# Aedelon/MASt3R-SLAM

Hardware: AMD Instinct MI355X
Metric: keyframe-pairs/sec (512x512 two-view infer+match+GN) (higher is better)
Workload: dtype fp16

## Files before the change

### mast3r-slam_amd/csrc/conv_tail.hip

```cpp
#include "gemm_common.h"

using namespace m3gemm;

namespace {

constexpr int kThreads = 512;
constexpr int TH = 16, TW = 32;
constexpr int HH = TH + 2, HW = TW + 2;
constexpr int kHaloPix = HH * HW;
constexpr int kHaloBytes = kHaloPix * 128;
constexpr int kWStage = 128 * 128;
constexpr int PH = 11, PW = 19;
constexpr int kPatchBytes = (PH * PW * 128 + 1023) / 1024 * 1024;
constexpr int kLdsBytes = kHaloBytes + 2 * kWStage + kPatchBytes;

struct TailArgs {
    const bf16_t *X;
    const bf16_t *Wc;
    const float *bias;
    const bf16_t *W4;
    const float *b4;
    float *pts, *conf;
    bf16_t *Y;
    const bf16_t *R;
    int cout, relu_in;
    const bf16_t *zero16;
    int B, H, W, IH, IW;
    const bf16_t *Wc2, *W42;
    const float *bias2, *b42;
};

enum { EP_PLAIN = 0 , EP_TAIL = 1 , EP_RELU = 2 ,
       EP_ADD = 3  };

template <int DT, bool UPS, int CIN, int EP>
__global__ void __launch_bounds__(kThreads, 2)
k_conv_tail(const TailArgs ain) {
    constexpr bool TAIL = EP == EP_TAIL;
    static_assert(CIN % 64 == 0 && (TAIL ? CIN == 128 : true), "64-channel steps; the fused tail is the 128-channel head.2");
    constexpr int NQ = CIN / 64;
    TailArgs a = ain;
    if (blockIdx.y == 1) {
        a.Wc = ain.Wc2; a.W4 = ain.W42; a.bias = ain.bias2; a.b4 = ain.b42;
        a.X = ain.X + (size_t)ain.B * ain.IH * ain.IW * CIN;
        if (TAIL) {
            a.pts = ain.pts + (size_t)ain.B * ain.H * ain.W * 3;
            a.conf = ain.conf + (size_t)ain.B * ain.H * ain.W;
        } else {
            a.Y = ain.Y + (size_t)ain.B * ain.H * ain.W * ain.cout;
            if (EP == EP_ADD) a.R = ain.R + (size_t)ain.B * ain.H * ain.W * ain.cout;
        }
    }
    if (!TAIL) {
        const int z = blockIdx.z;
        a.Wc += (size_t)z * 128 * 9 * CIN;
        if (a.bias) a.bias += z * 128;
        a.Y += z * 128;
        if (EP == EP_ADD) a.R += z * 128;
    }
    extern __shared__ __attribute__((aligned(16))) unsigned char lds[];
    unsigned char *halo = lds, *wst = lds + kHaloBytes, *patch = lds + kHaloBytes + 2 * kWStage;
    const int tid = threadIdx.x, lane = tid & 63, wave = tid >> 6;
    const int wp = wave >> 1, wc = wave & 1;
    const int tiles_x = (a.W + TW - 1) / TW, tiles_y = a.H / TH;
    const int nwg = tiles_x * tiles_y * a.B;
    const int bid = xcd_remap(blockIdx.x, nwg);
    const int b = bid / (tiles_x * tiles_y), trem = bid - b * tiles_x * tiles_y;
    const int ty = trem / tiles_x, tx = trem - ty * tiles_x;
    const int oy0 = ty * TH, ox0 = tx * TW;
    const bf16_t *img = a.X + (size_t)b * a.IH * a.IW * CIN;

    auto stage_w = [&](int tap, int half, int buf) {
        unsigned char *base = wst + buf * kWStage;
#pragma unroll
        for (int i = 0; i < 2; ++i) {
            const int slot = i * kThreads + tid;
            const int row = slot >> 3, cp = slot & 7;
            const int c = half * 8 + (cp ^ ((row >> 1) & 7));
            glds16(a.Wc + ((size_t)row * 9 + tap) * CIN + c * 8, base + i * (kThreads * 16) + wave * 1024);
        }
    };
    const float sy = UPS && a.H > 1 ? (float)(a.IH - 1) / (float)(a.H - 1) : 0.f;
    const float sx = UPS && a.W > 1 ? (float)(a.IW - 1) / (float)(a.W - 1) : 0.f;
    const int py0 = (int)((float)max(oy0 - 1, 0) * sy), px0 = (int)((float)max(ox0 - 1, 0) * sx);
    auto stage_patch = [&](int half) {
        for (int wi = wave; wi < (PH * PW * 8 + 63) / 64; wi += kThreads / 64) {
            int slot = wi * 64 + lane;
            slot = slot < PH * PW * 8 ? slot : PH * PW * 8 - 1;
            const int pp = slot >> 3, c = slot & 7;
            const int y = min(py0 + pp / PW, a.IH - 1), x = min(px0 + pp % PW, a.IW - 1);
            glds16(img + ((size_t)y * a.IW + x) * CIN + (half * 8 + c) * 8, patch + wi * 1024);
        }
    };
    auto stage_halo_direct = [&](int half) {
        for (int wi = wave; wi < (kHaloPix * 8 + 63) / 64; wi += kThreads / 64) {
            int slot = wi * 64 + lane;
            const bool live = slot < kHaloPix * 8;
            slot = live ? slot : kHaloPix * 8 - 1;
            const int pix = slot >> 3, cp = slot & 7;
            const int hy = pix / HW, hx = pix - hy * HW;
            const int iy = oy0 + hy - 1, ix = ox0 + hx - 1;
            const int c = half * 8 + (cp ^ ((hx >> 1) & 7));
            const bool in = iy >= 0 && iy < a.H && ix >= 0 && ix < a.W;
            const void *src = in ? (const void *)(img + ((size_t)iy * a.IW + ix) * CIN + c * 8) : (const void *)a.zero16;
            if (wi * 64 + 64 <= kHaloPix * 8) glds16(src, halo + wi * 1024);
            else if (live) *reinterpret_cast<uint4 *>(halo + (size_t)slot * 16) = *reinterpret_cast<const uint4 *>(src);
        }
    };
    auto blend_halo = [&]() {
        for (int slot = tid; slot < kHaloPix * 8; slot += kThreads) {
            const int pix = slot >> 3, cp = slot & 7;
            const int hy = pix / HW, hx = pix - hy * HW;
            const int iy = oy0 + hy - 1, ix = ox0 + hx - 1;
            const int c = cp ^ ((hx >> 1) & 7);
            uint4 o = make_uint4(0u, 0u, 0u, 0u);
            if (iy >= 0 && iy < a.H && ix >= 0 && ix < a.W) {
                const float fy = iy * sy, fx = ix * sx;
                int y0 = (int)fy, x0 = (int)fx;
                y0 = min(y0, a.IH - 1); x0 = min(x0, a.IW - 1);
                const int y1 = min(y0 + 1, a.IH - 1), x1 = min(x0 + 1, a.IW - 1);
                const float wy = fy - (float)y0, wx = fx - (float)x0;
                const unsigned char *p = patch + c * 16;
                union U { uint4 q; unsigned w[4]; } q00, q01, q10, q11, r;
                q00.q = *reinterpret_cast<const uint4 *>(p + ((y0 - py0) * PW + (x0 - px0)) * 128);
                q01.q = *reinterpret_cast<const uint4 *>(p + ((y0 - py0) * PW + (x1 - px0)) * 128);
                q10.q = *reinterpret_cast<const uint4 *>(p + ((y1 - py0) * PW + (x0 - px0)) * 128);
                q11.q = *reinterpret_cast<const uint4 *>(p + ((y1 - py0) * PW + (x1 - px0)) * 128);
#pragma unroll
                for (int k = 0; k < 4; ++k) {
                    const float tl = lo16<DT>(q00.w[k]) * (1.f - wx) + lo16<DT>(q01.w[k]) * wx;
                    const float bl = lo16<DT>(q10.w[k]) * (1.f - wx) + lo16<DT>(q11.w[k]) * wx;
                    const float th = hi16<DT>(q00.w[k]) * (1.f - wx) + hi16<DT>(q01.w[k]) * wx;
                    const float bh = hi16<DT>(q10.w[k]) * (1.f - wx) + hi16<DT>(q11.w[k]) * wx;
                    r.w[k] = pack16<DT>(tl * (1.f - wy) + bl * wy, th * (1.f - wy) + bh * wy);
                }
                o = r.q;
            }
            *reinterpret_cast<uint4 *>(halo + (size_t)slot * 16) = o;
        }
    };

    f32x4 acc[8][4];
#pragma unroll
    for (int i = 0; i < 8; ++i)
#pragma unroll
        for (int j = 0; j < 4; ++j) acc[i][j] = f32x4{0.f, 0.f, 0.f, 0.f};
    const int frow = lane & 15, fch = lane >> 4;
    int w_off[4];
#pragma unroll
    for (int j = 0; j < 4; ++j) {
        const int r = wc * 64 + j * 16 + frow;
        w_off[j] = r * 128 + ((fch ^ ((r >> 1) & 7)) << 4);
    }

    const int group = wave >> 2;
    bf16x8 af[8], wf[4];
    const int pix_of_row = (int)((0x3D9F2A40E6C851B7ULL >> (4 * frow)) & 15);
    auto col_offset = [&](int hx) { return hx * 128 + ((fch ^ ((hx >> 1) & 7)) << 4); };
    auto read_frags = [&](int g, int tap, int ks) {
        const int ky = tap / 3, kx = tap - ky * 3;
        const unsigned char *wsrc = wst + (g & 1) * kWStage;
        const int flip = ks << 6;
        const int c0 = col_offset(pix_of_row + kx) ^ flip;
        const int c1 = col_offset(16 + pix_of_row + kx) ^ flip;
        const unsigned char *rowp = halo + (wp * 4 + ky) * (HW * 128);
#pragma unroll
        for (int j = 0; j < 4; ++j) wf[j] = *reinterpret_cast<const bf16x8 *>(wsrc + (w_off[j] ^ flip));
#pragma unroll
        for (int i = 0; i < 8; ++i)
            af[i] = *reinterpret_cast<const bf16x8 *>(rowp + (i >> 1) * (HW * 128) + ((i & 1) ? c1 : c0));
        if (!TAIL && a.relu_in) {
#pragma unroll
            for (int i = 0; i < 8; ++i) af[i] = relu_frag(af[i]);
        }
    };
    auto mfma_all = [&]() {
        __builtin_amdgcn_s_setprio(1);
#pragma unroll
        for (int i = 0; i < 8; ++i)
#pragma unroll
            for (int j = 0; j < 4; ++j) acc[i][j] = mfma16<DT>(wf[j], af[i], acc[i][j]);
        __builtin_amdgcn_s_setprio(0);
    };
    auto phase_end = [&]() {
        __builtin_amdgcn_sched_barrier(0);
        __builtin_amdgcn_s_barrier();
        __builtin_amdgcn_sched_barrier(0);
    };
    auto phase_end_wait = [&]() {
        __builtin_amdgcn_sched_barrier(0);
        asm volatile("s_waitcnt vmcnt(0)" ::: "memory");
        __builtin_amdgcn_s_barrier();
        __builtin_amdgcn_sched_barrier(0);
    };
    auto prefetch_w = [&](int g) { if (g + 1 < 9 * NQ) stage_w((g + 1) % 9, (g + 1) / 9, (g + 1) & 1); };
    auto run_half = [&](int half) {
        if (group == 0) {
#pragma unroll 1
            for (int tap = 0; tap < 9; ++tap) {
                const int g = half * 9 + tap;
                read_frags(g, tap, 0);
                prefetch_w(g);
                asm volatile("s_waitcnt lgkmcnt(0)" ::: "memory");
                phase_end();
                mfma_all();
                phase_end();
                read_frags(g, tap, 1);
                asm volatile("s_waitcnt lgkmcnt(0)" ::: "memory");
                phase_end();
                mfma_all();
                phase_end_wait();
            }
            phase_end();
        } else {
#pragma unroll 1
            for (int tap = 0; tap < 9; ++tap) {
                const int g = half * 9 + tap;
                if (tap > 0) mfma_all();
                phase_end();
                read_frags(g, tap, 0);
                prefetch_w(g);
                asm volatile("s_waitcnt lgkmcnt(0)" ::: "memory");
                phase_end();
                mfma_all();
                phase_end();
                read_frags(g, tap, 1);
                asm volatile("s_waitcnt lgkmcnt(0)" ::: "memory");
                phase_end_wait();
            }
            mfma_all();
            phase_end();
        }
    };

    stage_w(0, 0, 0);
    if (UPS) stage_patch(0); else stage_halo_direct(0);
    asm volatile("s_waitcnt vmcnt(0)" ::: "memory");
    lds_barrier();
#pragma unroll 1
    for (int q = 0; q < NQ; ++q) {
        if (UPS) {
            blend_halo();
            lds_barrier();
            if (q + 1 < NQ) stage_patch(q + 1);
        } else if (q > 0) {
            stage_halo_direct(q);
            asm volatile("s_waitcnt vmcnt(0)" ::: "memory");
            lds_barrier();
        }
        run_half(q);
    }

    if constexpr (EP == EP_ADD) {
        const int r = lane & 15, gq = lane >> 4;
        constexpr int RS = 272;
        unsigned char *wl = halo + wave * (32 * RS);
        float4 bj[4];
#pragma unroll
        for (int j = 0; j < 4; ++j)
            bj[j] = a.bias ? *reinterpret_cast<const float4 *>(a.bias + wc * 64 + j * 16 + gq * 4) : make_float4(0.f, 0.f, 0.f, 0.f);
        auto pix = [&](int pass, int rl, int &oy, int &ox) {
            const int i = pass * 2 + (rl >> 4);
            oy = oy0 + wp * 4 + (i >> 1);
            ox = ox0 + (i & 1) * 16 + (int)((0x3D9F2A40E6C851B7ULL >> (4 * (rl & 15))) & 15);
        };
        uint4 q[2][4];
        auto load_resid = [&](int pass, uint4 (&dst)[4]) {
#pragma unroll
            for (int it = 0; it < 4; ++it) {
                const int c = it * 64 + lane, rl = c >> 3, ch = c & 7;
                int oy, ox;
                pix(pass, rl, oy, ox);
                ox = ox < a.W ? ox : a.W - 1;
                dst[it] = *reinterpret_cast<const uint4 *>(a.R + (((size_t)b * a.H + oy) * a.W + ox) * a.cout + wc * 64 + ch * 8);
            }
        };
        load_resid(0, q[0]);
#pragma unroll
        for (int pass = 0; pass < 4; ++pass) {
            if (pass + 1 < 4) load_resid(pass + 1, q[(pass + 1) & 1]);
#pragma unroll
            for (int ii = 0; ii < 2; ++ii)
#pragma unroll
                for (int j = 0; j < 4; ++j) {
                    const f32x4 v = acc[pass * 2 + ii][j];
                    *reinterpret_cast<float4 *>(wl + (ii * 16 + r) * RS + ((j * 4 + gq) << 4)) =
                        make_float4(v[0] + bj[j].x, v[1] + bj[j].y, v[2] + bj[j].z, v[3] + bj[j].w);
                }
            asm volatile("s_waitcnt lgkmcnt(0)" ::: "memory");
#pragma unroll
            for (int it = 0; it < 4; ++it) {
                const int c = it * 64 + lane, rl = c >> 3, ch = c & 7;
                const float4 f0 = *reinterpret_cast<const float4 *>(wl + rl * RS + ch * 32);
                const float4 f1 = *reinterpret_cast<const float4 *>(wl + rl * RS + ch * 32 + 16);
                const uint4 u = q[pass & 1][it];
                uint4 o;
                o.x = pack16<DT>(f0.x + lo16<DT>(u.x), f0.y + hi16<DT>(u.x));
                o.y = pack16<DT>(f0.z + lo16<DT>(u.y), f0.w + hi16<DT>(u.y));
                o.z = pack16<DT>(f1.x + lo16<DT>(u.z), f1.y + hi16<DT>(u.z));
                o.w = pack16<DT>(f1.z + lo16<DT>(u.w), f1.w + hi16<DT>(u.w));
                int oy, ox;
                pix(pass, rl, oy, ox);
                if (ox < a.W)
                    *reinterpret_cast<uint4 *>(a.Y + (((size_t)b * a.H + oy) * a.W + ox) * a.cout + wc * 64 + ch * 8) = o;
            }
            asm volatile("" ::: "memory");
        }
    } else if constexpr (!TAIL) {
        const int r = lane & 15, gq = lane >> 4;
        unsigned char *wl = halo + wave * 8192;
        float4 bj[4];
#pragma unroll
        for (int j = 0; j < 4; ++j)
            bj[j] = a.bias ? *reinterpret_cast<const float4 *>(a.bias + wc * 64 + j * 16 + gq * 4) : make_float4(0.f, 0.f, 0.f, 0.f);
#pragma unroll
        for (int pass = 0; pass < 2; ++pass) {
#pragma unroll
            for (int ii = 0; ii < 4; ++ii)
#pragma unroll
                for (int j = 0; j < 4; ++j) {
                    f32x4 v = acc[pass * 4 + ii][j];
                    v[0] += bj[j].x; v[1] += bj[j].y; v[2] += bj[j].z; v[3] += bj[j].w;
                    if (EP == EP_RELU) {
#pragma unroll
                        for (int e = 0; e < 4; ++e) v[e] = v[e] > 0.f ? v[e] : 0.f;
                    }
                    uint2 pk;
                    pk.x = pack16<DT>(v[0], v[1]); pk.y = pack16<DT>(v[2], v[3]);
                    *reinterpret_cast<uint2 *>(wl + (ii * 16 + r) * 128 + (((j * 2 + (gq >> 1)) ^ ((r >> 1) & 7)) << 4) + (((gq ^ r) & 1) << 3)) = pk;
                }
            asm volatile("s_waitcnt lgkmcnt(0)" ::: "memory");
#pragma unroll
            for (int it = 0; it < 8; ++it) {
                const int c = it * 64 + lane, rl = c >> 3, ch = c & 7;
                uint4 v = *reinterpret_cast<const uint4 *>(wl + rl * 128 + ((ch ^ ((rl >> 1) & 7)) << 4));
                if (rl & 1) v = uint4{v.z, v.w, v.x, v.y};
                const int i = pass * 4 + (rl >> 4);
                const int oy = oy0 + wp * 4 + (i >> 1);
                const int ox = ox0 + (i & 1) * 16 + (int)((0x3D9F2A40E6C851B7ULL >> (4 * (rl & 15))) & 15);
                if (ox < a.W)
                    *reinterpret_cast<uint4 *>(a.Y + (((size_t)b * a.H + oy) * a.W + ox) * a.cout + wc * 64 + ch * 8) = v;
            }
            asm volatile("" ::: "memory");
        }
    } else {
        const int r = lane & 15, gq = lane >> 4;
        float part[8][4];
    #pragma unroll
        for (int i = 0; i < 8; ++i)
    #pragma unroll
            for (int o = 0; o < 4; ++o) part[i][o] = 0.f;
    #pragma unroll
        for (int j = 0; j < 4; ++j) {
            const int n = wc * 64 + j * 16 + gq * 4;
            const float4 bq = a.bias ? *reinterpret_cast<const float4 *>(a.bias + n) : make_float4(0.f, 0.f, 0.f, 0.f);
            float w4[4][4];
    #pragma unroll
            for (int o = 0; o < 4; ++o) {
                const uint2 q = *reinterpret_cast<const uint2 *>(a.W4 + (size_t)o * 128 + n);
                w4[o][0] = lo16<DT>(q.x); w4[o][1] = hi16<DT>(q.x); w4[o][2] = lo16<DT>(q.y); w4[o][3] = hi16<DT>(q.y);
            }
    #pragma unroll
            for (int i = 0; i < 8; ++i) {
                const f32x4 v = acc[i][j];
                const float h[4] = {fmaxf(v[0] + bq.x, 0.f), fmaxf(v[1] + bq.y, 0.f), fmaxf(v[2] + bq.z, 0.f), fmaxf(v[3] + bq.w, 0.f)};
    #pragma unroll
                for (int o = 0; o < 4; ++o)
                    part[i][o] += (h[0] * w4[o][0] + h[1] * w4[o][1]) + (h[2] * w4[o][2] + h[3] * w4[o][3]);
            }
        }
    #pragma unroll
        for (int i = 0; i < 8; ++i)
    #pragma unroll
            for (int o = 0; o < 4; ++o) {
                float v = part[i][o];
                v += __shfl_xor(v, 16, 64);
                v += __shfl_xor(v, 32, 64);
                part[i][o] = v;
            }
        float *red = reinterpret_cast<float *>(wst);
        if (gq == 0) {
    #pragma unroll
            for (int i = 0; i < 8; ++i)
                *reinterpret_cast<float4 *>(red + (((wp * 2 + wc) * 8 + i) * 16 + r) * 4) = make_float4(part[i][0], part[i][1], part[i][2], part[i][3]);
        }
        __syncthreads();
        {
            const int i = 4 * wc + gq;
            const float4 p0 = *reinterpret_cast<const float4 *>(red + (((wp * 2 + 0) * 8 + i) * 16 + r) * 4);
            const float4 p1 = *reinterpret_cast<const float4 *>(red + (((wp * 2 + 1) * 8 + i) * 16 + r) * 4);
            const int oy = oy0 + wp * 4 + (i >> 1), ox = ox0 + (i & 1) * 16 + pix_of_row;
            if (ox < a.W) {
                const float x = p0.x + p1.x + a.b4[0], y = p0.y + p1.y + a.b4[1];
                const float z = p0.z + p1.z + a.b4[2], c = p0.w + p1.w + a.b4[3];
                const float d = sqrtf(x * x + y * y + z * z);
                const float sc = expm1f(d) / fmaxf(d, 1e-8f);
                const size_t m = ((size_t)b * a.H + oy) * a.W + ox;
                a.pts[3 * m + 0] = x * sc; a.pts[3 * m + 1] = y * sc; a.pts[3 * m + 2] = z * sc;
                a.conf[m] = 1.0f + expf(c);
            }
        }
    }
}

}

extern "C" {

static int dpt_tail_launch(const void *X, const void *Wc, const float *bias, const void *W4, const float *b4,
                           const void *Wc2, const float *bias2, const void *W42, const float *b42, float *pts,
                           float *conf, void *Y, const void *R, const void *zero16, int B, int H, int W, int cin, int cout,
                           int ep, int relu_in, int upsample, int dtype, void *stream) {
    const int groups = Wc2 ? 2 : 1;
    const bool tail = ep == EP_TAIL;
    M3_REQUIRE(X && Wc && zero16 && B > 0 && H > 0 && W > 0 && H % 16 == 0 && W % 16 == 0);
    M3_REQUIRE(tail ? (W4 && b4 && pts && conf && cin == 128 && !Y)
                    : (Y && (cin == 128 || cin == 256) && (cout == 128 || cout == 256) && (ep == EP_PLAIN || ep == EP_RELU || ep == EP_ADD)));
    M3_REQUIRE((ep == EP_ADD) == (R != nullptr) && (!upsample || ep == EP_PLAIN || tail));
    M3_REQUIRE(groups == 1 || ((!tail || (W42 && b42)) && (bias == nullptr) == (bias2 == nullptr)));
    M3_REQUIRE((dtype == DT_BF16 || dtype == DT_F16) && (!upsample || (H % 2 == 0 && W % 2 == 0)));
    M3_REQUIRE((int64_t)groups * B * H * W < (1ll << 31));
    M3_REQUIRE(reinterpret_cast<uintptr_t>(X) % 16 == 0 && reinterpret_cast<uintptr_t>(Wc) % 16 == 0 &&
               reinterpret_cast<uintptr_t>(Y) % 16 == 0 && reinterpret_cast<uintptr_t>(R) % 16 == 0);
    TailArgs a;
    a.Wc2 = (const bf16_t *)Wc2; a.W42 = (const bf16_t *)W42; a.bias2 = bias2; a.b42 = b42;
    a.X = (const bf16_t *)X; a.Wc = (const bf16_t *)Wc; a.bias = bias; a.W4 = (const bf16_t *)W4; a.b4 = b4;
    a.pts = pts; a.conf = conf; a.Y = (bf16_t *)Y; a.R = (const bf16_t *)R; a.cout = tail ? 128 : cout; a.relu_in = relu_in;
    a.zero16 = (const bf16_t *)zero16; a.B = B; a.H = H; a.W = W;
    a.IH = upsample ? H / 2 : H; a.IW = upsample ? W / 2 : W;
    const dim3 grid((unsigned)((H / TH) * ((W + TW - 1) / TW) * B), groups, tail ? 1 : cout / 128), blk(kThreads);
    hipStream_t st = (hipStream_t)stream;
#define M3_TAIL(DTV, UP, CI, EPV)                                                                                \
    do {                                                                                                         \
        static M3AttrOnce once;                                                                                  \
        int dev__;                                                                                               \
        if (m3_attr_need(once, &dev__)) {                                                                        \
            M3_CHECK_HIP(hipFuncSetAttribute(reinterpret_cast<const void *>(&k_conv_tail<DTV, UP, CI, EPV>),     \
                                             hipFuncAttributeMaxDynamicSharedMemorySize, kLdsBytes), "m3_dpt_tail/attr"); \
            m3_attr_done(once, dev__);                                                                           \
        }                                                                                                        \
        hipLaunchKernelGGL((k_conv_tail<DTV, UP, CI, EPV>), grid, blk, kLdsBytes, st, a);                        \
    } while (0)
#define M3_TAIL_DT(UP, CI, EPV) do { if (dtype == DT_F16) M3_TAIL(DT_F16, UP, CI, EPV); else M3_TAIL(DT_BF16, UP, CI, EPV); } while (0)
    if (tail) { if (upsample) M3_TAIL_DT(true, 128, EP_TAIL); else M3_TAIL_DT(false, 128, EP_TAIL); }
    else if (ep == EP_PLAIN && cin == 128) { if (upsample) M3_TAIL_DT(true, 128, EP_PLAIN); else M3_TAIL_DT(false, 128, EP_PLAIN); }
    else if (ep == EP_PLAIN) { if (upsample) M3_TAIL_DT(true, 256, EP_PLAIN); else M3_TAIL_DT(false, 256, EP_PLAIN); }
    else if (ep == EP_RELU) { if (cin == 128) M3_TAIL_DT(false, 128, EP_RELU); else M3_TAIL_DT(false, 256, EP_RELU); }
    else { if (cin == 128) M3_TAIL_DT(false, 128, EP_ADD); else M3_TAIL_DT(false, 256, EP_ADD); }
#undef M3_TAIL_DT
#undef M3_TAIL
    M3_CHECK_LAUNCH("m3_dpt_tail");
    return M3_OK;
}

int m3_dpt_tail_grouped2_dt(const void *X, const void *Wc0, const void *Wc1, const float *bias0, const float *bias1,
                            const void *W40, const void *W41, const float *b40, const float *b41, float *pts,
                            float *conf, const void *zero16, int B, int H, int W, int upsample, int dtype, void *stream) {
    M3_REQUIRE(pts && conf && (Wc1 == nullptr) == (W41 == nullptr));
    if (!Wc1) bias1 = b41 = nullptr;
    return dpt_tail_launch(X, Wc0, bias0, W40, b40, Wc1, bias1, W41, b41, pts, conf, nullptr, nullptr, zero16, B, H, W, 128, 128,
                           EP_TAIL, 0, upsample, dtype, stream);
}

int m3_conv3x3_up_direct_grouped2_dt(const void *X, const void *Wc0, const void *Wc1, const float *bias0, const float *bias1,
                                     void *Y, const void *zero16, int B, int H, int W, int Cin, int upsample, int dtype,
                                     void *stream) {
    M3_REQUIRE(Y != nullptr);
    return dpt_tail_launch(X, Wc0, bias0, nullptr, nullptr, Wc1, Wc1 ? bias1 : nullptr, nullptr, nullptr, nullptr, nullptr, Y,
                           nullptr, zero16, B, H, W, Cin, 128, EP_PLAIN, 0, upsample, dtype, stream);
}

int m3_conv3x3_direct_grouped2_dt(const void *X, const void *W0, const void *W1, const float *bias0, const float *bias1,
                                  void *Y, const void *R, const void *zero16, int B, int H, int W, int Cin, int Cout,
                                  int epilogue, int dtype, void *stream) {
    const int relu_in = (epilogue & 0x100) ? 1 : 0;
    const int e = epilogue & 0xff;
    M3_REQUIRE(Y != nullptr && (e == M3_EPI_BF16 || e == M3_EPI_BF16_RELU || e == M3_EPI_BF16_ADD));
    const int ep = e == M3_EPI_BF16 ? EP_PLAIN : (e == M3_EPI_BF16_RELU ? EP_RELU : EP_ADD);
    return dpt_tail_launch(X, W0, bias0, nullptr, nullptr, W1, bias1, nullptr, nullptr, nullptr, nullptr, Y, R, zero16, B, H, W,
                           Cin, Cout, ep, relu_in, 0, dtype, stream);
}

}
```

Measured before the change: 295.4.

## Make conv tail kernel persistent with cross-tile weight and patch prefetch

Turns the 3D grid of conv tiles into a persistent 1D grid sized to the CU count, with each workgroup looping over items (tile × group × cout-slice). The last weight step and the next upsample patch are prefetched for the following item, so loads overlap the current tile's tail. The tail reduction scratch moves from the weight stage buffer to the halo buffer so the prefetched weights are not overwritten. Compile-time ablation switches are also added. The risks are that only one workgroup runs per CU although launch bounds allow two, more address arithmetic per item, and a loss of latency hiding from concurrent blocks.

New measurement: 294.4. About the same (-0.3%).

```diff
diff --git a/mast3r-slam_amd/csrc/conv_tail.hip b/mast3r-slam_amd/csrc/conv_tail.hip
--- a/mast3r-slam_amd/csrc/conv_tail.hip
+++ b/mast3r-slam_amd/csrc/conv_tail.hip
@@ -13,6 +13,11 @@
 constexpr int PH = 11, PW = 19;
 constexpr int kPatchBytes = (PH * PW * 128 + 1023) / 1024 * 1024;
 constexpr int kLdsBytes = kHaloBytes + 2 * kWStage + kPatchBytes;
+
+#ifndef M3_TAIL_ABLATE
+#define M3_TAIL_ABLATE 0
+#endif
+constexpr bool kStage = !(M3_TAIL_ABLATE & 1), kEpilogue = !(M3_TAIL_ABLATE & 2), kPersistent = !(M3_TAIL_ABLATE & 4);
 
 struct TailArgs {
     const bf16_t *X;
@@ -26,6 +31,7 @@
     int cout, relu_in;
     const bf16_t *zero16;
     int B, H, W, IH, IW;
+    int groups;
     const bf16_t *Wc2, *W42;
     const float *bias2, *b42;
 };
@@ -39,57 +45,89 @@
     constexpr bool TAIL = EP == EP_TAIL;
     static_assert(CIN % 64 == 0 && (TAIL ? CIN == 128 : true), "64-channel steps; the fused tail is the 128-channel head.2");
     constexpr int NQ = CIN / 64;
-    TailArgs a = ain;
-    if (blockIdx.y == 1) {
-        a.Wc = ain.Wc2; a.W4 = ain.W42; a.bias = ain.bias2; a.b4 = ain.b42;
-        a.X = ain.X + (size_t)ain.B * ain.IH * ain.IW * CIN;
-        if (TAIL) {
-            a.pts = ain.pts + (size_t)ain.B * ain.H * ain.W * 3;
-            a.conf = ain.conf + (size_t)ain.B * ain.H * ain.W;
-        } else {
-            a.Y = ain.Y + (size_t)ain.B * ain.H * ain.W * ain.cout;
-            if (EP == EP_ADD) a.R = ain.R + (size_t)ain.B * ain.H * ain.W * ain.cout;
-        }
-    }
-    if (!TAIL) {
-        const int z = blockIdx.z;
-        a.Wc += (size_t)z * 128 * 9 * CIN;
-        if (a.bias) a.bias += z * 128;
-        a.Y += z * 128;
-        if (EP == EP_ADD) a.R += z * 128;
-    }
+    static_assert((9 * NQ) % 2 == 0, "a tile's first weight step lands in stage 0 again: the last step prefetches it for the next tile");
     extern __shared__ __attribute__((aligned(16))) unsigned char lds[];
     unsigned char *halo = lds, *wst = lds + kHaloBytes, *patch = lds + kHaloBytes + 2 * kWStage;
-    const int tid = threadIdx.x, lane = tid & 63, wave = tid >> 6;
-    const int wp = wave >> 1, wc = wave & 1;
-    const int tiles_x = (a.W + TW - 1) / TW, tiles_y = a.H / TH;
-    const int nwg = tiles_x * tiles_y * a.B;
-    const int bid = xcd_remap(blockIdx.x, nwg);
-    const int b = bid / (tiles_x * tiles_y), trem = bid - b * tiles_x * tiles_y;
-    const int ty = trem / tiles_x, tx = trem - ty * tiles_x;
-    const int oy0 = ty * TH, ox0 = tx * TW;
-    const bf16_t *img = a.X + (size_t)b * a.IH * a.IW * CIN;
-
-    auto stage_w = [&](int tap, int half, int buf) {
+    int tid = threadIdx.x, lane, wave, wp, wc;
+    int frow, fch, group, pix_of_row, w_off[4];
+    auto derive = [&]() {
+        asm volatile("" : "+v"(tid));
+        lane = tid & 63; wave = tid >> 6;
+        wp = wave >> 1; wc = wave & 1;
+        frow = lane & 15; fch = lane >> 4;
+        group = wave >> 2;
+        pix_of_row = (int)((0x3D9F2A40E6C851B7ULL >> (4 * frow)) & 15);
+#pragma unroll
+        for (int j = 0; j < 4; ++j) {
+            const int r = wc * 64 + j * 16 + frow;
+            w_off[j] = r * 128 + ((fch ^ ((r >> 1) & 7)) << 4);
+        }
+    };
+    derive();
+    const int tiles_x = (ain.W + TW - 1) / TW, tiles_y = ain.H / TH;
+    const int ntile = tiles_x * tiles_y * ain.B, nz = TAIL ? 1 : ain.cout / 128;
+    const int nitem = ntile * ain.groups * nz;
+    const float sy = UPS && ain.H > 1 ? (float)(ain.IH - 1) / (float)(ain.H - 1) : 0.f;
+    const float sx = UPS && ain.W > 1 ? (float)(ain.IW - 1) / (float)(ain.W - 1) : 0.f;
+    struct Item { const bf16_t *Wc, *img; int grp, z, b, oy0, ox0, py0, px0; };
+    auto locate = [&](int item) {
+        Item t;
+        const int bid = xcd_remap(item, nitem);
+        const int gz = bid / ntile, trem0 = bid - gz * ntile;
+        t.grp = gz / nz; t.z = gz - t.grp * nz;
+        t.b = trem0 / (tiles_x * tiles_y);
+        const int trem = trem0 - t.b * tiles_x * tiles_y;
+        const int ty = trem / tiles_x, tx = trem - ty * tiles_x;
+        t.oy0 = ty * TH; t.ox0 = tx * TW;
+        t.py0 = (int)((float)max(t.oy0 - 1, 0) * sy); t.px0 = (int)((float)max(t.ox0 - 1, 0) * sx);
+        t.Wc = (t.grp ? ain.Wc2 : ain.Wc) + (size_t)t.z * 128 * 9 * CIN;
+        t.img = ain.X + ((size_t)t.grp * ain.B + t.b) * ain.IH * ain.IW * CIN;
+        return t;
+    };
+    int item = blockIdx.x;
+    bool has_next = false;
+    struct { const bf16_t *Wc, *W4, *R; bf16_t *Y; const float *bias, *b4; float *pts, *conf; } a;
+    int b = 0, oy0 = 0, ox0 = 0;
+    const bf16_t *img = nullptr;
+    auto enter = [&](const Item &t) {
+        a.Wc = ain.Wc; a.W4 = ain.W4; a.bias = ain.bias; a.b4 = ain.b4;
+        a.pts = ain.pts; a.conf = ain.conf; a.Y = ain.Y; a.R = ain.R;
+        if (t.grp == 1) {
+            a.Wc = ain.Wc2; a.W4 = ain.W42; a.bias = ain.bias2; a.b4 = ain.b42;
+            if (TAIL) {
+                a.pts = ain.pts + (size_t)ain.B * ain.H * ain.W * 3;
+                a.conf = ain.conf + (size_t)ain.B * ain.H * ain.W;
+            } else {
+                a.Y = ain.Y + (size_t)ain.B * ain.H * ain.W * ain.cout;
+                if (EP == EP_ADD) a.R = ain.R + (size_t)ain.B * ain.H * ain.W * ain.cout;
+            }
+        }
+        if (!TAIL) {
+            a.Wc += (size_t)t.z * 128 * 9 * CIN;
+            if (a.bias) a.bias += t.z * 128;
+            a.Y += t.z * 128;
+            if (EP == EP_ADD) a.R += t.z * 128;
+        }
+        b = t.b; oy0 = t.oy0; ox0 = t.ox0; img = t.img;
+    };
+
+    auto stage_w = [&](const bf16_t *Wc, int tap, int half, int buf) {
         unsigned char *base = wst + buf * kWStage;
 #pragma unroll
         for (int i = 0; i < 2; ++i) {
             const int slot = i * kThreads + tid;
             const int row = slot >> 3, cp = slot & 7;
             const int c = half * 8 + (cp ^ ((row >> 1) & 7));
-            glds16(a.Wc + ((size_t)row * 9 + tap) * CIN + c * 8, base + i * (kThreads * 16) + wave * 1024);
-        }
-    };
-    const float sy = UPS && a.H > 1 ? (float)(a.IH - 1) / (float)(a.H - 1) : 0.f;
-    const float sx = UPS && a.W > 1 ? (float)(a.IW - 1) / (float)(a.W - 1) : 0.f;
-    const int py0 = (int)((float)max(oy0 - 1, 0) * sy), px0 = (int)((float)max(ox0 - 1, 0) * sx);
-    auto stage_patch = [&](int half) {
+            glds16(Wc + ((size_t)row * 9 + tap) * CIN + c * 8, base + i * (kThreads * 16) + wave * 1024);
+        }
+    };
+    auto stage_patch = [&](const Item &t, int half) {
         for (int wi = wave; wi < (PH * PW * 8 + 63) / 64; wi += kThreads / 64) {
             int slot = wi * 64 + lane;
             slot = slot < PH * PW * 8 ? slot : PH * PW * 8 - 1;
             const int pp = slot >> 3, c = slot & 7;
-            const int y = min(py0 + pp / PW, a.IH - 1), x = min(px0 + pp % PW, a.IW - 1);
-            glds16(img + ((size_t)y * a.IW + x) * CIN + (half * 8 + c) * 8, patch + wi * 1024);
+            const int y = min(t.py0 + pp / PW, ain.IH - 1), x = min(t.px0 + pp % PW, ain.IW - 1);
+            glds16(t.img + ((size_t)y * ain.IW + x) * CIN + (half * 8 + c) * 8, patch + wi * 1024);
         }
     };
     auto stage_halo_direct = [&](int half) {
@@ -101,24 +139,25 @@
             const int hy = pix / HW, hx = pix - hy * HW;
             const int iy = oy0 + hy - 1, ix = ox0 + hx - 1;
             const int c = half * 8 + (cp ^ ((hx >> 1) & 7));
-            const bool in = iy >= 0 && iy < a.H && ix >= 0 && ix < a.W;
-            const void *src = in ? (const void *)(img + ((size_t)iy * a.IW + ix) * CIN + c * 8) : (const void *)a.zero16;
+            const bool in = iy >= 0 && iy < ain.H && ix >= 0 && ix < ain.W;
+            const void *src = in ? (const void *)(img + ((size_t)iy * ain.IW + ix) * CIN + c * 8) : (const void *)ain.zero16;
             if (wi * 64 + 64 <= kHaloPix * 8) glds16(src, halo + wi * 1024);
             else if (live) *reinterpret_cast<uint4 *>(halo + (size_t)slot * 16) = *reinterpret_cast<const uint4 *>(src);
         }
     };
     auto blend_halo = [&]() {
+        const int py0 = (int)((float)max(oy0 - 1, 0) * sy), px0 = (int)((float)max(ox0 - 1, 0) * sx);
         for (int slot = tid; slot < kHaloPix * 8; slot += kThreads) {
             const int pix = slot >> 3, cp = slot & 7;
             const int hy = pix / HW, hx = pix - hy * HW;
             const int iy = oy0 + hy - 1, ix = ox0 + hx - 1;
             const int c = cp ^ ((hx >> 1) & 7);
             uint4 o = make_uint4(0u, 0u, 0u, 0u);
-            if (iy >= 0 && iy < a.H && ix >= 0 && ix < a.W) {
+            if (iy >= 0 && iy < ain.H && ix >= 0 && ix < ain.W) {
                 const float fy = iy * sy, fx = ix * sx;
                 int y0 = (int)fy, x0 = (int)fx;
-                y0 = min(y0, a.IH - 1); x0 = min(x0, a.IW - 1);
-                const int y1 = min(y0 + 1, a.IH - 1), x1 = min(x0 + 1, a.IW - 1);
+                y0 = min(y0, ain.IH - 1); x0 = min(x0, ain.IW - 1);
+                const int y1 = min(y0 + 1, ain.IH - 1), x1 = min(x0 + 1, ain.IW - 1);
                 const float wy = fy - (float)y0, wx = fx - (float)x0;
                 const unsigned char *p = patch + c * 16;
                 union U { uint4 q; unsigned w[4]; } q00, q01, q10, q11, r;
@@ -141,21 +180,8 @@
     };
 
     f32x4 acc[8][4];
-#pragma unroll
-    for (int i = 0; i < 8; ++i)
-#pragma unroll
-        for (int j = 0; j < 4; ++j) acc[i][j] = f32x4{0.f, 0.f, 0.f, 0.f};
-    const int frow = lane & 15, fch = lane >> 4;
-    int w_off[4];
-#pragma unroll
-    for (int j = 0; j < 4; ++j) {
-        const int r = wc * 64 + j * 16 + frow;
-        w_off[j] = r * 128 + ((fch ^ ((r >> 1) & 7)) << 4);
-    }
-
-    const int group = wave >> 2;
+
     bf16x8 af[8], wf[4];
-    const int pix_of_row = (int)((0x3D9F2A40E6C851B7ULL >> (4 * frow)) & 15);
     auto col_offset = [&](int hx) { return hx * 128 + ((fch ^ ((hx >> 1) & 7)) << 4); };
     auto read_frags = [&](int g, int tap, int ks) {
         const int ky = tap / 3, kx = tap - ky * 3;
@@ -169,7 +195,7 @@
 #pragma unroll
         for (int i = 0; i < 8; ++i)
             af[i] = *reinterpret_cast<const bf16x8 *>(rowp + (i >> 1) * (HW * 128) + ((i & 1) ? c1 : c0));
-        if (!TAIL && a.relu_in) {
+        if (!TAIL && ain.relu_in) {
 #pragma unroll
             for (int i = 0; i < 8; ++i) af[i] = relu_frag(af[i]);
         }
@@ -193,7 +219,13 @@
         __builtin_amdgcn_s_barrier();
         __builtin_amdgcn_sched_barrier(0);
     };
-    auto prefetch_w = [&](int g) { if (g + 1 < 9 * NQ) stage_w((g + 1) % 9, (g + 1) / 9, (g + 1) & 1); };
+    auto prefetch_w = [&](int g) {
+        const bool wrap = g + 1 == 9 * NQ;
+        if (wrap && !has_next) return;
+        const bf16_t *Wc = wrap ? locate(item + (int)gridDim.x).Wc : a.Wc;
+        const int g1 = wrap ? 0 : g + 1;
+        stage_w(Wc, g1 % 9, g1 / 9, g1 & 1);
+    };
     auto run_half = [&](int half) {
         if (group == 0) {
 #pragma unroll 1
@@ -233,24 +265,43 @@
         }
     };
 
-    stage_w(0, 0, 0);
-    if (UPS) stage_patch(0); else stage_halo_direct(0);
+    enter(locate(item));
+    stage_w(a.Wc, 0, 0, 0);
+    if (kStage) { if (UPS) stage_patch(locate(item), 0); else stage_halo_direct(0); }
     asm volatile("s_waitcnt vmcnt(0)" ::: "memory");
     lds_barrier();
 #pragma unroll 1
+    for (;;) {
+    has_next = item + (int)gridDim.x < nitem;
+    derive();
+#pragma unroll
+    for (int i = 0; i < 8; ++i)
+#pragma unroll
+        for (int j = 0; j < 4; ++j) acc[i][j] = f32x4{0.f, 0.f, 0.f, 0.f};
+#pragma unroll 1
     for (int q = 0; q < NQ; ++q) {
         if (UPS) {
-            blend_halo();
+            if (kStage) blend_halo();
             lds_barrier();
-            if (q + 1 < NQ) stage_patch(q + 1);
+            if (kStage) { if (q + 1 < NQ) stage_patch(locate(item), q + 1); else if (has_next) stage_patch(locate(item + (int)gridDim.x), 0); }
         } else if (q > 0) {
-            stage_halo_direct(q);
+            if (kStage) stage_halo_direct(q);
             asm volatile("s_waitcnt vmcnt(0)" ::: "memory");
             lds_barrier();
         }
         run_half(q);
     }
 
+    if constexpr (!kEpilogue) {
+        if (ain.B < 0) {
+            float sum = 0.f;
+#pragma unroll
+            for (int i = 0; i < 8; ++i)
+#pragma unroll
+                for (int j = 0; j < 4; ++j) sum += acc[i][j][0] + acc[i][j][1] + acc[i][j][2] + acc[i][j][3];
+            if (TAIL) a.conf[tid] = sum; else a.Y[tid] = (bf16_t)pack16<DT>(sum, sum);
+        }
+    } else
     if constexpr (EP == EP_ADD) {
         const int r = lane & 15, gq = lane >> 4;
         constexpr int RS = 272;
@@ -271,8 +322,8 @@
                 const int c = it * 64 + lane, rl = c >> 3, ch = c & 7;
                 int oy, ox;
                 pix(pass, rl, oy, ox);
-                ox = ox < a.W ? ox : a.W - 1;
-                dst[it] = *reinterpret_cast<const uint4 *>(a.R + (((size_t)b * a.H + oy) * a.W + ox) * a.cout + wc * 64 + ch * 8);
+                ox = ox < ain.W ? ox : ain.W - 1;
+                dst[it] = *reinterpret_cast<const uint4 *>(a.R + (((size_t)b * ain.H + oy) * ain.W + ox) * ain.cout + wc * 64 + ch * 8);
             }
         };
         load_resid(0, q[0]);
@@ -301,8 +352,8 @@
                 o.w = pack16<DT>(f1.z + lo16<DT>(u.w), f1.w + hi16<DT>(u.w));
                 int oy, ox;
                 pix(pass, rl, oy, ox);
-                if (ox < a.W)
-                    *reinterpret_cast<uint4 *>(a.Y + (((size_t)b * a.H + oy) * a.W + ox) * a.cout + wc * 64 + ch * 8) = o;
+                if (ox < ain.W)
+                    *reinterpret_cast<uint4 *>(a.Y + (((size_t)b * ain.H + oy) * ain.W + ox) * ain.cout + wc * 64 + ch * 8) = o;
             }
             asm volatile("" ::: "memory");
         }
@@ -338,8 +389,8 @@
                 const int i = pass * 4 + (rl >> 4);
                 const int oy = oy0 + wp * 4 + (i >> 1);
                 const int ox = ox0 + (i & 1) * 16 + (int)((0x3D9F2A40E6C851B7ULL >> (4 * (rl & 15))) & 15);
-                if (ox < a.W)
-                    *reinterpret_cast<uint4 *>(a.Y + (((size_t)b * a.H + oy) * a.W + ox) * a.cout + wc * 64 + ch * 8) = v;
+                if (ox < ain.W)
+                    *reinterpret_cast<uint4 *>(a.Y + (((size_t)b * ain.H + oy) * ain.W + ox) * ain.cout + wc * 64 + ch * 8) = v;
             }
             asm volatile("" ::: "memory");
         }
@@ -378,7 +429,7 @@
                 v += __shfl_xor(v, 32, 64);
                 part[i][o] = v;
             }
-        float *red = reinterpret_cast<float *>(wst);
+        float *red = reinterpret_cast<float *>(halo);
         if (gq == 0) {
     #pragma unroll
             for (int i = 0; i < 8; ++i)
@@ -389,17 +440,28 @@
             const int i = 4 * wc + gq;
             const float4 p0 = *reinterpret_cast<const float4 *>(red + (((wp * 2 + 0) * 8 + i) * 16 + r) * 4);
             const float4 p1 = *reinterpret_cast<const float4 *>(red + (((wp * 2 + 1) * 8 + i) * 16 + r) * 4);
-            const int oy = oy0 + wp * 4 + (i >> 1), ox = ox0 + (i & 1) * 16 + pix_of_row;
-            if (ox < a.W) {
+            const int oy = oy0 + wp * 4 + (i >> 1), ox = ox0 + (i & 1) * 16 + (int)((0x3D9F2A40E6C851B7ULL >> (4 * r)) & 15);
+            if (ox < ain.W) {
                 const float x = p0.x + p1.x + a.b4[0], y = p0.y + p1.y + a.b4[1];
                 const float z = p0.z + p1.z + a.b4[2], c = p0.w + p1.w + a.b4[3];
                 const float d = sqrtf(x * x + y * y + z * z);
                 const float sc = expm1f(d) / fmaxf(d, 1e-8f);
-                const size_t m = ((size_t)b * a.H + oy) * a.W + ox;
+                const size_t m = ((size_t)b * ain.H + oy) * ain.W + ox;
                 a.pts[3 * m + 0] = x * sc; a.pts[3 * m + 1] = y * sc; a.pts[3 * m + 2] = z * sc;
                 a.conf[m] = 1.0f + expf(c);
             }
         }
+    }
+
+    if (!has_next) break;
+    lds_barrier();
+    item += (int)gridDim.x;
+    enter(locate(item));
+    if (!UPS) {
+        if (kStage) stage_halo_direct(0);
+        asm volatile("s_waitcnt vmcnt(0)" ::: "memory");
+        lds_barrier();
+    }
     }
 }
 
@@ -428,7 +490,11 @@
     a.pts = pts; a.conf = conf; a.Y = (bf16_t *)Y; a.R = (const bf16_t *)R; a.cout = tail ? 128 : cout; a.relu_in = relu_in;
     a.zero16 = (const bf16_t *)zero16; a.B = B; a.H = H; a.W = W;
     a.IH = upsample ? H / 2 : H; a.IW = upsample ? W / 2 : W;
-    const dim3 grid((unsigned)((H / TH) * ((W + TW - 1) / TW) * B), groups, tail ? 1 : cout / 128), blk(kThreads);
+    a.groups = groups;
+    const int nitem = (H / TH) * ((W + TW - 1) / TW) * B * groups * (tail ? 1 : cout / 128);
+    const int cus = m3_device_cu_count();
+    M3_REQUIRE(cus > 0);
+    const dim3 grid((unsigned)(kPersistent && nitem > cus ? cus : nitem)), blk(kThreads);
     hipStream_t st = (hipStream_t)stream;
 #define M3_TAIL(DTV, UP, CI, EPV)                                                                                \
     do {                                                                                                         \
```
